# b0nes164/GPUSorting

Hardware: AMD Instinct MI355X
Metric: GKeys/s uint32 OneSweep at 1/2/4/8 MI355X; % HBM-read roofline (higher is better)
Workload: dtype u32; 1 GPU; 2^28 uniform-random uint32 keys-only OneSweep, 1 MI355X (BASELINE configs[1]); keys_per_gpu=268435456, entropy_preset=1, generator=InitRandom seed 10+i (+1000*rank), tile_keys=16384, verified_sorted=True

## Files before the change

### gpusorting_amd/csrc/hybrid_kernels.hpp

```cpp
#pragma once
#include "onesweep_kernels.hpp"
#include "mid_kernels.hpp"

namespace gs {

constexpr uint32_t HY_BINS = 65536;
constexpr uint32_t HY_JOINT_WORDS = HY_BINS / 2;
constexpr uint32_t HY_SLICE_WORDS = HY_JOINT_WORDS + RADIX;
constexpr uint32_t HY_VALID = 0;
constexpr uint32_t HY_MAXBUCKET = 1;
constexpr uint32_t HYT_JOINT = 0;
constexpr uint32_t HYT_BASE = HY_BINS;
constexpr uint32_t HYT_T = HYT_BASE + HY_BINS + 64;
constexpr uint32_t HYT_WORDS = HYT_T + NCH * RADIX;
static_assert(HYT_BASE % 4 == 0 && HYT_T % 4 == 0, "16-byte accesses");

constexpr int HY_HIST_THREADS = 1024;
constexpr uint32_t HY_FOLD_CHUNKS = 256;

template <int KT>
__global__ __launch_bounds__(HY_HIST_THREADS, HY_HIST_THREADS / 256) void hy_histogram_kernel(
    const uint32_t* __restrict__ keys, uint32_t* slab, size_t slab_used_words, uint32_t n, uint32_t seg_len0, uint32_t per_wg,
    uint32_t wg_per_seg, uint32_t* slices, uint32_t cap ) {
    static_assert(KeyWords<KT>::value == 1, "32-bit keys");
    constexpr uint32_t T = HY_HIST_THREADS;
    __shared__ __attribute__((aligned(16))) uint32_t s_j[HY_JOINT_WORDS];
    __shared__ __attribute__((aligned(16))) uint32_t s_r[RADIX / 2 * 32];
    __shared__ uint32_t s_b0[RADIX];
    __shared__ uint32_t s_red[4];
    const uint32_t tid = threadIdx.x, lane = tid & 63u;
    uint32_t* hist = slab + SLAB_HIST;
    {
        uint4* a = reinterpret_cast<uint4*>(slab);
        const size_t na = SLAB_HIST / 4, b0 = SLAB_HSUB / 4, nb = slab_used_words / 4;
        const size_t stride = (size_t)gridDim.x * T;
        const uint4 z = {0u, 0u, 0u, 0u};
        for (size_t i = (size_t)blockIdx.x * T + tid; i < na; i += stride) a[i] = z;
        for (size_t i = b0 + (size_t)blockIdx.x * T + tid; i < nb; i += stride) a[i] = z;
    }
    for (uint32_t i = tid; i < HY_JOINT_WORDS / 4; i += T) reinterpret_cast<uint4*>(s_j)[i] = uint4{0u, 0u, 0u, 0u};
    for (uint32_t i = tid; i < RADIX / 2 * 32 / 4; i += T) reinterpret_cast<uint4*>(s_r)[i] = uint4{0u, 0u, 0u, 0u};
    if (tid < RADIX) s_b0[tid] = 0;
    if (tid < 4) s_red[tid] = 0;
    auto fold = [&]() {
        __syncthreads();
        for (uint32_t i = tid; i < RADIX / 2 * 8; i += T) {
            const uint4 v = reinterpret_cast<const uint4*>(s_r)[i];
            reinterpret_cast<uint4*>(s_r)[i] = uint4{0u, 0u, 0u, 0u};
            uint32_t lo = (v.x & 0xffffu) + (v.y & 0xffffu) + (v.z & 0xffffu) + (v.w & 0xffffu);
            uint32_t hi = (v.x >> 16) + (v.y >> 16) + (v.z >> 16) + (v.w >> 16);
#pragma unroll
            for (int m = 1; m < 8; m <<= 1) {
                lo += __shfl_xor(lo, m, 64);
                hi += __shfl_xor(hi, m, 64);
            }
            if ((i & 7u) == 0u) {
                s_b0[(i >> 3) * 2u] += lo;
                s_b0[(i >> 3) * 2u + 1u] += hi;
            }
        }
        __syncthreads();
    };
    __syncthreads();

    const uint32_t x = blockIdx.x / wg_per_seg, jr = blockIdx.x % wg_per_seg;
    const unsigned long long sb = (unsigned long long)x * seg_len0, se = sb + seg_len0;
    const uint32_t seg_begin = sb < n ? (uint32_t)sb : n, seg_end = se < n ? (uint32_t)se : n;
    const unsigned long long rb = (unsigned long long)seg_begin + (unsigned long long)jr * per_wg;
    const uint32_t begin = rb < seg_end ? (uint32_t)rb : seg_end;
    const uint32_t end = (unsigned long long)begin + per_wg < seg_end ? begin + per_wg : seg_end;

    uint32_t k_or = 0, k_nand = 0;
    bool skew = false;
    uint32_t sticky = 0xffffffffu;
    uint32_t since_fold = 0;
    bool joint_off = false;
    typedef uint32_t hv4 __attribute__((ext_vector_type(4)));
    auto ld16 = [](const uint32_t* q) -> uint4 {
        const hv4 v = __builtin_nontemporal_load(reinterpret_cast<const hv4*>(q));
        return uint4{v.x, v.y, v.z, v.w};
    };
    auto add_joint = [&](uint32_t p, uint32_t c) { atomicAdd(&s_j[p >> 1], c << ((p & 1u) << 4)); };
    auto process = [&](const uint4 t, const bool probe) {
        const uint32_t b[4] = {t.x, t.y, t.z, t.w};
        k_or |= t.x | t.y | t.z | t.w;
        k_nand |= ~(t.x & t.y & t.z & t.w);
        if (since_fold >= HY_FOLD_CHUNKS) {
            fold();
            since_fold = 0;
        }
        ++since_fold;
#pragma unroll
        for (int j = 0; j < 4; ++j) {
            const uint32_t d = b[j] & 255u;
            atomicAdd(&s_r[(d >> 1) * 32u + (lane & 31u)], 1u << ((d & 1u) * 16u));
        }
        if (joint_off) return;
        if (probe) {
            const uint32_t p0 = b[0] >> 16;
            const uint32_t f = (uint32_t)__builtin_amdgcn_readfirstlane((int)p0);
            const uint32_t pc = (uint32_t)__popcll(__builtin_amdgcn_ballot_w64(p0 == f));
            if (pc >= HIST_SKEW_LANES) {
                skew = true;
                if (pc >= 24 || sticky == 0xffffffffu) sticky = f;
            }
        }
        if (!skew) {
#pragma unroll
            for (int j = 0; j < 4; ++j) add_joint(b[j] >> 16, 1u);
            return;
        }
        const uint32_t f = (uint32_t)__builtin_amdgcn_readfirstlane((int)(b[0] >> 16));
        const uint32_t pc = (uint32_t)__popcll(__builtin_amdgcn_ballot_w64((b[0] >> 16) == f));
        if (pc >= 24 && f != sticky) sticky = f;
        if (__builtin_amdgcn_ballot_w64((b[0] >> 16) == sticky && (b[1] >> 16) == sticky && (b[2] >> 16) == sticky && (b[3] >> 16) == sticky) == ~0ull) {
            if (lane == 0) add_joint(sticky, 256u);
            return;
        }
        uint32_t hit = 0;
#pragma unroll
        for (int j = 0; j < 4; ++j) {
            const uint32_t p = b[j] >> 16;
            const unsigned long long m = __builtin_amdgcn_ballot_w64(p == sticky);
            hit += (uint32_t)__popcll(m);
            if (p != sticky) add_joint(p, 1u);
            else if (__builtin_amdgcn_mbcnt_hi((uint32_t)(m >> 32), __builtin_amdgcn_mbcnt_lo((uint32_t)m, 0u)) == 0u)
                add_joint(sticky, (uint32_t)__popcll(m));
        }
        if (hit < 32) {
            sticky = f;
            if (pc < 8) skew = false;
        }
    };
    constexpr uint32_t UNROLL = HY_HIST_UNROLL;
    for (uint32_t c0 = begin; c0 < end; c0 += UNROLL * HIST_CHUNK) {
        if ((unsigned long long)c0 + UNROLL * HIST_CHUNK <= end) {
            uint4 t[UNROLL];
#pragma unroll
            for (uint32_t u = 0; u < UNROLL; ++u) t[u] = ld16(keys + c0 + u * HIST_CHUNK + tid * 4u);
            if (!joint_off) {
                const uint32_t pf = to_bits<KT>((uint32_t)__builtin_amdgcn_readfirstlane((int)t[0].x)) >> 16;
                if (lane == 0 && (((s_j[pf >> 1] >> ((pf & 1u) << 4)) & 0xffffu) > cap ||
                                  (skew && ((s_j[sticky >> 1] >> ((sticky & 1u) << 4)) & 0xffffu) > cap))) s_red[3] = 1u;
                joint_off = __builtin_amdgcn_readfirstlane((int)s_red[3]) != 0;
            }
#pragma unroll
            for (uint32_t u = 0; u < UNROLL; ++u)
                process(uint4{to_bits<KT>(t[u].x), to_bits<KT>(t[u].y), to_bits<KT>(t[u].z), to_bits<KT>(t[u].w)}, u == 0);
            continue;
        }
        for (uint32_t c = c0; c < end; c += HIST_CHUNK) {
            if ((unsigned long long)c + HIST_CHUNK <= end) {
                const uint4 t = ld16(keys + c + tid * 4u);
                process(uint4{to_bits<KT>(t.x), to_bits<KT>(t.y), to_bits<KT>(t.z), to_bits<KT>(t.w)}, true);
            } else {
                for (uint32_t i = c + tid; i < end; i += T) {
                    const uint32_t kb = to_bits<KT>(keys[i]);
                    k_or |= kb;
                    k_nand |= ~kb;
                    add_joint(kb >> 16, 1u);
                    atomicAdd(&s_b0[kb & 255u], 1u);
                }
            }
        }
    }
    fold();
    uint32_t* mine = slices + (size_t)blockIdx.x * HY_SLICE_WORDS;
    uint32_t sum = 0;
    for (uint32_t i = tid; i < HY_JOINT_WORDS / 4; i += T) {
        const uint4 v = reinterpret_cast<const uint4*>(s_j)[i];
        reinterpret_cast<uint4*>(mine)[i] = v;
        sum += (v.x & 0xffffu) + (v.x >> 16) + (v.y & 0xffffu) + (v.y >> 16) + (v.z & 0xffffu) + (v.z >> 16) + (v.w & 0xffffu) + (v.w >> 16);
    }
    if (tid < RADIX) mine[HY_JOINT_WORDS + tid] = s_b0[tid];
    sum = wave_reduce_sum(sum);
#pragma unroll
    for (int dd = 32; dd > 0; dd >>= 1) {
        k_or |= __shfl_xor(k_or, dd, 64);
        k_nand |= __shfl_xor(k_nand, dd, 64);
    }
    if (lane == 0) {
        atomicAdd(&s_red[0], sum);
        atomicOr(&s_red[1], k_or);
        atomicOr(&s_red[2], k_nand);
    }
    __syncthreads();
    if (tid == 0) {
        if (s_red[0] != end - begin || s_red[3] != 0u) atomicOr(&hist[HIST_TABLE_WORDS + HX_HY_BAD], 1u);
        atomicOr(&hist[HIST_TABLE_WORDS + HX_OR], s_red[1]);
        atomicOr(&hist[HIST_TABLE_WORDS + HX_NAND], s_red[2]);
    }
}

__global__ __launch_bounds__(256) void hy_reduce_kernel(const uint32_t* __restrict__ slices, uint32_t G, uint32_t wg_per_seg,
                                                         uint32_t* __restrict__ tab, uint32_t* __restrict__ hist) {
    __shared__ uint32_t s_acc[RADIX], s_T[NCH];
    const uint32_t tid = threadIdx.x;
    if (blockIdx.x >= RADIX) {
        const uint32_t x = blockIdx.x - RADIX;
        uint32_t acc = 0;
        for (uint32_t w = x * wg_per_seg; w < (x + 1u) * wg_per_seg && w < G; ++w) acc += slices[(size_t)w * HY_SLICE_WORDS + HY_JOINT_WORDS + tid];
        hist[hist_index(0, tid, x)] = acc;
        return;
    }
    const uint32_t b3 = blockIdx.x, w4 = tid & 31u, grp = tid >> 5;
    s_acc[tid] = 0;
    if (tid < NCH) s_T[tid] = 0;
    __syncthreads();
    uint32_t a[8] = {0u, 0u, 0u, 0u, 0u, 0u, 0u, 0u}, cur_x = 0xffffffffu, acc_x = 0;
    constexpr uint32_t U = 16;
    for (uint32_t s0 = grp; s0 < G; s0 += 8u * U) {
        uint4 v[U];
#pragma unroll
        for (uint32_t k = 0; k < U; ++k) {
            const uint32_t sl = s0 + 8u * k;
            v[k] = *reinterpret_cast<const uint4*>(slices + (size_t)(sl < G ? sl : G - 1u) * HY_SLICE_WORDS + b3 * 128u + w4 * 4u);
        }
#pragma unroll
        for (uint32_t k = 0; k < U; ++k) {
            const uint32_t sl = s0 + 8u * k;
            if (sl < G) {
                const uint32_t xs = sl / wg_per_seg;
                if (xs != cur_x) {
                    if (acc_x) atomicAdd(&s_T[cur_x], acc_x);
                    cur_x = xs;
                    acc_x = 0;
                }
                const uint32_t h[8] = {v[k].x & 0xffffu, v[k].x >> 16, v[k].y & 0xffffu, v[k].y >> 16, v[k].z & 0xffffu, v[k].z >> 16, v[k].w & 0xffffu, v[k].w >> 16};
#pragma unroll
                for (int j = 0; j < 8; ++j) { a[j] += h[j]; acc_x += h[j]; }
            }
        }
    }
    if (acc_x) atomicAdd(&s_T[cur_x], acc_x);
#pragma unroll
    for (int j = 0; j < 8; ++j) atomicAdd(&s_acc[w4 * 8u + j], a[j]);
    __syncthreads();
    tab[HYT_JOINT + b3 * RADIX + tid] = s_acc[tid];
    if (tid < NCH) tab[HYT_T + tid * RADIX + b3] = s_T[tid];
}

__global__ __launch_bounds__(1024) void hy_scan_kernel(uint32_t* slab, uint32_t* tab, uint32_t n, uint32_t seg_len0, uint32_t desc_stride,
                                                        uint32_t cap, uint32_t tile, uint32_t pregrouped ) {
    __shared__ uint32_t s_wt[RADIX];
    __shared__ uint32_t s_wmax[16], s_c4[4], s_rw[4];
    __shared__ uint32_t s_bstart[RADIX + 1], s_rowbase[RADIX];
    const uint32_t tid = threadIdx.x, lane = tid & 63u, wave = tid >> 6;
    uint32_t* hist = slab + SLAB_HIST;
    uint4 v[16];
#pragma unroll
    for (int i = 0; i < 16; ++i) v[i] = reinterpret_cast<const uint4*>(tab + HYT_JOINT)[i * 1024 + tid];
    uint32_t incl[16], mx = 0;
#pragma unroll
    for (int i = 0; i < 16; ++i) {
        const uint32_t s4 = v[i].x + v[i].y + v[i].z + v[i].w;
        const uint32_t m01 = v[i].x > v[i].y ? v[i].x : v[i].y, m23 = v[i].z > v[i].w ? v[i].z : v[i].w, m = m01 > m23 ? m01 : m23;
        mx = m > mx ? m : mx;
        incl[i] = wave_inclusive_scan_dpp(s4);
        if (lane == 63) s_wt[i * 16 + wave] = incl[i];
    }
#pragma unroll
    for (int dd = 32; dd > 0; dd >>= 1) {
        const uint32_t o = (uint32_t)__shfl_xor((int)mx, dd, 64);
        mx = o > mx ? o : mx;
    }
    if (lane == 0) s_wmax[wave] = mx;
    __syncthreads();
    uint32_t cv = 0, cincl = 0;
    if (tid < RADIX) {
        cv = s_wt[tid];
        cincl = wave_inclusive_scan_dpp(cv);
        if (lane == 63) s_c4[wave] = cincl;
    }
    __syncthreads();
    uint32_t total = 0, maxb = 0;
    for (uint32_t w = 0; w < 4; ++w) total += s_c4[w];
    for (uint32_t w = 0; w < 16; ++w) maxb = s_wmax[w] > maxb ? s_wmax[w] : maxb;
    if (tid < RADIX) {
        uint32_t b = cincl - cv;
        for (uint32_t w = 0; w < wave; ++w) b += s_c4[w];
        s_wt[tid] = b;
    }
    const bool valid = hist[HIST_TABLE_WORDS + HX_HY_BAD] == 0u && maxb <= cap && total == n;
    if (tid == 0) slab[SLAB_HY + HY_MAXBUCKET] = maxb;
    if (!valid) {
        if (tid == 0) hist[HIST_TABLE_WORDS + HX_SKEW] = 1u;
        return;
    }
    __syncthreads();
    uint32_t tseg[NCH];
#pragma unroll
    for (uint32_t x = 0; x < NCH; ++x) tseg[x] = tid < RADIX ? tab[HYT_T + x * RADIX + tid] : 0u;
#pragma unroll
    for (int i = 0; i < 16; ++i) {
        const uint4 c = v[i];
        const uint32_t e = s_wt[i * 16 + wave] + incl[i] - (c.x + c.y + c.z + c.w);
        v[i] = uint4{e, e + c.x, e + c.x + c.y, e + c.x + c.y + c.z};
        reinterpret_cast<uint4*>(tab + HYT_BASE)[i * 1024 + tid] = v[i];
        if (lane == 0) s_bstart[i * 16 + wave] = e;
    }
    if (tid == 0) {
        s_bstart[RADIX] = n;
        tab[HYT_BASE + HY_BINS] = n;
    }
    __syncthreads();
    uint32_t* info0 = slab + SLAB_INFO;
    uint32_t* info1 = info0 + INFO_STRIDE;
    uint32_t* desc0 = slab + SLAB_DESC;
    uint32_t* desc1 = desc0 + desc_stride;
    uint32_t rows = 0, rincl = 0;
    if (tid < RADIX) {
        rows = chain_tiles(s_bstart[tid], s_bstart[tid + 1], tile) + 1u;
        rincl = wave_inclusive_scan_dpp(rows);
        if (lane == 63) s_rw[wave] = rincl;
    }
    __syncthreads();
    if (tid < RADIX) {
        uint32_t rb = rincl - rows;
        for (uint32_t w = 0; w < wave; ++w) rb += s_rw[w];
        s_rowbase[tid] = rb;
        info1[I_START + tid] = s_bstart[tid];
        info1[I_END + tid] = s_bstart[tid + 1];
        info1[I_ROW + tid] = rb;
    }
    __syncthreads();
#pragma unroll
    for (int i = 0; i < 16; ++i) {
        uint4* row = reinterpret_cast<uint4*>(desc1 + (size_t)s_rowbase[i * 16 + wave] * RADIX);
        row[lane] = uint4{(v[i].x << 2) | FLAG_INCLUSIVE, (v[i].y << 2) | FLAG_INCLUSIVE, (v[i].z << 2) | FLAG_INCLUSIVE, (v[i].w << 2) | FLAG_INCLUSIVE};
    }
    if (tid < RADIX) {
        uint32_t run = s_bstart[tid], rowa = 0;
#pragma unroll
        for (uint32_t x = 0; x < NCH; ++x) {
            const unsigned long long a = (unsigned long long)x * seg_len0, b = a + seg_len0;
            const uint32_t s0 = a < n ? (uint32_t)a : n, s1 = b < n ? (uint32_t)b : n;
            desc0[(size_t)rowa * RADIX + tid] = (run << 2) | FLAG_INCLUSIVE;
            run += tseg[x];
            if (tid == 0) {
                info0[I_START + x] = s0;
                info0[I_END + x] = s1;
                info0[I_ROW + x] = rowa;
            }
            rowa += chain_tiles(s0, s1, tile) + 1u;
        }
    }
    if (tid == 0) {
        info0[PASS_FLAGS] = pregrouped ? PF_SKIP : 0u;
        info0[I_NCH] = NCH;
        info0[I_NEXT_SHIFT] = 0xffffffffu;
        info0[I_SHIFT] = 24u;
        info0[I_MODE] = 0xffffffffu;
        info1[PASS_FLAGS] = PF_SRC_ALT | PF_LAST;
        info1[I_NCH] = CHMAX;
        info1[I_NEXT_SHIFT] = 0xffffffffu;
        info1[I_SHIFT] = 16u;
        info1[I_MODE] = 0xffffffffu;
        info0[2 * INFO_STRIDE + PASS_FLAGS] = PF_SKIP;
        info0[3 * INFO_STRIDE + PASS_FLAGS] = PF_SKIP;
        hist[HIST_TABLE_WORDS + HX_HY] = 1u;
        slab[SLAB_HY + HY_VALID] = 1u;
    }
}
static_assert(CHMAX == RADIX, "pass B: one chain per top-byte value");

template <int KT, int THREADS_, int KPT_>
__global__ __launch_bounds__(THREADS_) void hy_local_sort_kernel(uint32_t* keys, const uint32_t* __restrict__ tab, uint32_t* __restrict__ slab,
                                                                 uint32_t n, uint32_t descending) {
    constexpr int KPT = KPT_, WAVES = THREADS_ / 64;
    constexpr uint32_t THREADS = THREADS_, TILE = THREADS_ * KPT_;
    static_assert(THREADS >= RADIX && KPT % 2 == 0 && WAVES % 2 == 0 && TILE < 65536, "one digit per thread in the scans; ranks and counters are packed two per word");
    __shared__ __attribute__((aligned(16))) uint32_t s_stage[TILE];
    __shared__ uint32_t s_cnt[WAVES / 2 * RADIX];
    __shared__ uint32_t s_wtot[4];
    const uint32_t tid = threadIdx.x, lane = tid & 63u, wave = tid >> 6;
    const uint32_t valid = slab[SLAB_HY + HY_VALID], b_lo = tab[HYT_BASE + blockIdx.x], b_hi = tab[HYT_BASE + blockIdx.x + 1u];
    if (__builtin_amdgcn_readfirstlane((int)valid) == 0) return;
    const uint32_t start = b_lo, count = b_hi - b_lo;
    if (count == 0u || count > TILE || start > n || count > n - start) return;
    const uint32_t at = descending ? n - start - count : start;
    const uint32_t kpt = (uint32_t)__builtin_amdgcn_readfirstlane((int)((count + THREADS - 1u) / THREADS));
    const uint32_t my_base = wave * (64u * kpt) + lane;
    uint32_t key[KPT];
#pragma unroll
    for (int i = 0; i < KPT; ++i) {
        if ((uint32_t)i >= kpt) continue;
        const uint32_t slot = my_base + i * 64u;
        key[i] = keys[at + (slot < count ? slot : count - 1u)];
    }
    if (tid < RADIX) s_cnt[tid] = 0;
#pragma unroll
    for (int i = 0; i < KPT; ++i)
        if ((uint32_t)i < kpt) key[i] = to_bits<KT>(key[i]);
    __syncthreads();
    uint32_t off[KPT / 2];
#pragma unroll
    for (int i = 0; i < KPT / 2; ++i) off[i] = 0;
#pragma unroll
    for (int i = 0; i < KPT; ++i) {
        if ((uint32_t)i >= kpt) continue;
        if (my_base + i * 64u < count)
            off[i >> 1] |= __hip_atomic_fetch_add(&s_cnt[key[i] & 255u], 1u, __ATOMIC_RELAXED, __HIP_MEMORY_SCOPE_WORKGROUP) << (16 * (i & 1));
    }
    __syncthreads();
    uint32_t c = 0, scan_incl = 0;
    if (tid < RADIX) {
        c = s_cnt[tid];
        scan_incl = wave_inclusive_scan_dpp(c);
        if (lane == 63) s_wtot[wave] = scan_incl;
    }
    __syncthreads();
    if (tid < RADIX) {
        uint32_t wbase = 0;
        for (uint32_t w = 0; w < wave; ++w) wbase += s_wtot[w];
        s_cnt[tid] = wbase + scan_incl - c;
    }
    __syncthreads();
#pragma unroll
    for (int i = 0; i < KPT; ++i) {
        if ((uint32_t)i >= kpt) continue;
        if (my_base + i * 64u < count) s_stage[((off[i >> 1] >> (16 * (i & 1))) & 0xffffu) + s_cnt[key[i] & 255u]] = key[i];
    }
    __syncthreads();
#pragma unroll
    for (int i = 0; i < KPT; ++i) {
        if ((uint32_t)i >= kpt) continue;
        key[i] = s_stage[my_base + i * 64u];
    }
    for (uint32_t i = tid; i < WAVES / 2 * RADIX; i += THREADS) s_cnt[i] = 0;
    __syncthreads();
    const uint32_t wsh = (uint32_t)__builtin_amdgcn_readfirstlane((int)((wave & 1u) * 16u));
    uint32_t* wh = s_cnt + (wave >> 1) * RADIX;
#pragma unroll
    for (int i = 0; i < KPT / 2; ++i) off[i] = 0;
#pragma unroll
    for (int i = 0; i < KPT; ++i) {
        if ((uint32_t)i >= kpt) continue;
        if (my_base + i * 64u < count) {
            const uint32_t r = __hip_atomic_fetch_add(&wh[(key[i] >> 8) & 255u], 1u << wsh, __ATOMIC_RELAXED, __HIP_MEMORY_SCOPE_WORKGROUP);
            off[i >> 1] |= ((r >> wsh) & 0xffffu) << (16 * (i & 1));
        }
    }
    __syncthreads();
    uint32_t run = 0;
    if (tid < RADIX) {
#pragma unroll
        for (int p = 0; p < WAVES / 2; ++p) {
            const uint32_t c2 = s_cnt[p * RADIX + tid];
            s_cnt[p * RADIX + tid] = run | ((run + (c2 & 0xffffu)) << 16);
            run += (c2 & 0xffffu) + (c2 >> 16);
        }
        scan_incl = wave_inclusive_scan_dpp(run);
        if (lane == 63) s_wtot[wave] = scan_incl;
    }
    __syncthreads();
    if (tid < RADIX) {
        uint32_t wbase = 0;
        for (uint32_t w = 0; w < wave; ++w) wbase += s_wtot[w];
        const uint32_t dpre = wbase + scan_incl - run;
#pragma unroll
        for (int p = 0; p < WAVES / 2; ++p) s_cnt[p * RADIX + tid] += dpre * 0x10001u;
    }
    __syncthreads();
#pragma unroll
    for (int i = 0; i < KPT; ++i) {
        if ((uint32_t)i >= kpt) continue;
        if (my_base + i * 64u < count)
            s_stage[((off[i >> 1] >> (16 * (i & 1))) & 0xffffu) + ((wh[(key[i] >> 8) & 255u] >> wsh) & 0xffffu)] = key[i];
    }
    __syncthreads();
#pragma unroll
    for (int i = 0; i < KPT; ++i) {
        const uint32_t slot = my_base + i * 64u;
        if ((uint32_t)i < kpt && slot < count) keys[at + (descending ? count - 1u - slot : slot)] = from_bits<KT>(s_stage[slot]);
    }
}

template <int KT, int VB, int THREADS_, int KPT_>
__global__ __launch_bounds__(THREADS_) void hy_local_sort_pairs_kernel(uint32_t* keys, void* vals_, const uint32_t* __restrict__ tab,
                                                                       const uint32_t* __restrict__ slab, uint32_t n, uint32_t descending) {
    using V = typename ValT<VB>::type;
    constexpr int KPT = KPT_, WAVES = THREADS_ / 64;
    constexpr uint32_t THREADS = THREADS_, TILE = THREADS_ * KPT_;
    static_assert(THREADS >= RADIX && KPT % 2 == 0 && WAVES % 2 == 0 && TILE < 65536, "slots of origin and counters are 16-bit fields");
    __shared__ __attribute__((aligned(16))) unsigned char s_raw[TILE * (VB > 4 ? VB : 4)];
    __shared__ uint32_t s_cnt[WAVES / 2 * RADIX];
    __shared__ uint32_t s_wtot[4];
    uint32_t* s_stage = reinterpret_cast<uint32_t*>(s_raw);
    V* s_vstage = reinterpret_cast<V*>(s_raw);
    V* vals = reinterpret_cast<V*>(vals_);
    const uint32_t tid = threadIdx.x, lane = tid & 63u, wave = tid >> 6;
    const uint32_t valid = slab[SLAB_HY + HY_VALID], b_lo = tab[HYT_BASE + blockIdx.x], b_hi = tab[HYT_BASE + blockIdx.x + 1u];
    if (__builtin_amdgcn_readfirstlane((int)valid) == 0) return;
    const uint32_t start = b_lo, count = b_hi - b_lo;
    if (count == 0u || count > TILE || start > n || count > n - start) return;
    const uint32_t at = descending ? n - start - count : start;
    const uint32_t kpt = (uint32_t)__builtin_amdgcn_readfirstlane((int)((count + THREADS - 1u) / THREADS));
    const uint32_t my_base = wave * (64u * kpt) + lane;
    uint32_t key[KPT];
    V val[KPT];
#pragma unroll
    for (int i = 0; i < KPT; ++i) {
        if ((uint32_t)i >= kpt) continue;
        const uint32_t slot = my_base + i * 64u, cs = slot < count ? slot : count - 1u;
        const uint32_t pos = at + (descending ? count - 1u - cs : cs);
        key[i] = keys[pos];
        val[i] = vals[pos];
    }
    const uint32_t wsh = (uint32_t)__builtin_amdgcn_readfirstlane((int)((wave & 1u) * 16u));
    uint32_t* wh = s_cnt + (wave >> 1) * RADIX;
#pragma unroll
    for (int i = 0; i < KPT; ++i)
        if ((uint32_t)i < kpt) key[i] = (to_bits<KT>(key[i]) & 0xffffu) | ((my_base + i * 64u) << 16);
    uint32_t off[KPT / 2];
#pragma unroll 1
    for (uint32_t shift = 0; shift < 16; shift += 8) {
        for (uint32_t i = tid; i < WAVES / 2 * RADIX; i += THREADS) s_cnt[i] = 0;
        __syncthreads();
#pragma unroll
        for (int i = 0; i < KPT / 2; ++i) off[i] = 0;
#pragma unroll
        for (int i = 0; i < KPT; ++i) {
            if ((uint32_t)i >= kpt) continue;
            if (my_base + i * 64u < count) {
                const uint32_t r = __hip_atomic_fetch_add(&wh[(key[i] >> shift) & 255u], 1u << wsh, __ATOMIC_RELAXED, __HIP_MEMORY_SCOPE_WORKGROUP);
                off[i >> 1] |= ((r >> wsh) & 0xffffu) << (16 * (i & 1));
            }
        }
        __syncthreads();
        uint32_t run = 0, scan_incl = 0;
        if (tid < RADIX) {
#pragma unroll
            for (int p = 0; p < WAVES / 2; ++p) {
                const uint32_t c2 = s_cnt[p * RADIX + tid];
                s_cnt[p * RADIX + tid] = run | ((run + (c2 & 0xffffu)) << 16);
                run += (c2 & 0xffffu) + (c2 >> 16);
            }
            scan_incl = wave_inclusive_scan_dpp(run);
            if (lane == 63) s_wtot[wave] = scan_incl;
        }
        __syncthreads();
        if (tid < RADIX) {
            uint32_t wbase = 0;
            for (uint32_t w = 0; w < wave; ++w) wbase += s_wtot[w];
            const uint32_t dpre = wbase + scan_incl - run;
#pragma unroll
            for (int p = 0; p < WAVES / 2; ++p) s_cnt[p * RADIX + tid] += dpre * 0x10001u;
        }
        __syncthreads();
#pragma unroll
        for (int i = 0; i < KPT; ++i) {
            if ((uint32_t)i >= kpt) continue;
            if (my_base + i * 64u < count)
                s_stage[((off[i >> 1] >> (16 * (i & 1))) & 0xffffu) + ((wh[(key[i] >> shift) & 255u] >> wsh) & 0xffffu)] = key[i];
        }
        __syncthreads();
#pragma unroll
        for (int i = 0; i < KPT; ++i) {
            if ((uint32_t)i >= kpt) continue;
            key[i] = s_stage[my_base + i * 64u];
        }
    }
    __syncthreads();
#pragma unroll
    for (int i = 0; i < KPT; ++i) {
        if ((uint32_t)i >= kpt) continue;
        if (my_base + i * 64u < count) s_vstage[my_base + i * 64u] = val[i];
    }
    __syncthreads();
    const uint32_t top = blockIdx.x << 16;
#pragma unroll
    for (int i = 0; i < KPT; ++i) {
        const uint32_t slot = my_base + i * 64u;
        if ((uint32_t)i < kpt && slot < count) {
            const uint32_t pos = at + (descending ? count - 1u - slot : slot);
            keys[pos] = from_bits<KT>(top | (key[i] & 0xffffu));
            vals[pos] = s_vstage[key[i] >> 16];
        }
    }
}

__global__ __launch_bounds__(256) void hy_void_copy_kernel(const uint32_t* __restrict__ slab, const uint4* __restrict__ src, uint4* __restrict__ dst,
                                                            size_t words16, const uint32_t* __restrict__ src_tail, uint32_t* __restrict__ dst_tail,
                                                            uint32_t tail_words) {
    if (__builtin_amdgcn_readfirstlane((int)slab[SLAB_HY + HY_VALID]) != 0) return;
    const size_t stride = (size_t)gridDim.x * 256u;
    for (size_t i = (size_t)blockIdx.x * 256u + threadIdx.x; i < words16; i += stride) dst[i] = src[i];
    if (blockIdx.x == 0 && threadIdx.x < tail_words) dst_tail[threadIdx.x] = src_tail[threadIdx.x];
}

}
```

Before: 167.7 GKeys/s.

## Stage only low 16 bits of keys in LDS during hybrid local sort

```diff
diff --git a/gpusorting_amd/csrc/hybrid_kernels.hpp b/gpusorting_amd/csrc/hybrid_kernels.hpp
--- a/gpusorting_amd/csrc/hybrid_kernels.hpp
+++ b/gpusorting_amd/csrc/hybrid_kernels.hpp
@@ -367,38 +367,40 @@
 template <int KT, int THREADS_, int KPT_>
 __global__ __launch_bounds__(THREADS_) void hy_local_sort_kernel(uint32_t* keys, const uint32_t* __restrict__ tab, uint32_t* __restrict__ slab,
                                                                  uint32_t n, uint32_t descending) {
-    constexpr int KPT = KPT_, WAVES = THREADS_ / 64;
+    constexpr int KPT = KPT_, KP2 = KPT_ / 2, WAVES = THREADS_ / 64;
     constexpr uint32_t THREADS = THREADS_, TILE = THREADS_ * KPT_;
-    static_assert(THREADS >= RADIX && KPT % 2 == 0 && WAVES % 2 == 0 && TILE < 65536, "one digit per thread in the scans; ranks and counters are packed two per word");
-    __shared__ __attribute__((aligned(16))) uint32_t s_stage[TILE];
+    static_assert(THREADS >= RADIX && KPT % 2 == 0 && WAVES % 2 == 0 && TILE < 65536 && TILE % 128 == 0,
+                  "one digit per thread in the scans; ranks and counters are packed two per word; the stage is whole blocks of 128 halfwords");
+    __shared__ __attribute__((aligned(16))) uint32_t s_stage[TILE / 2 + 4];
     __shared__ uint32_t s_cnt[WAVES / 2 * RADIX];
     __shared__ uint32_t s_wtot[4];
+    uint16_t* s_half = reinterpret_cast<uint16_t*>(s_stage);
     const uint32_t tid = threadIdx.x, lane = tid & 63u, wave = tid >> 6;
     const uint32_t valid = slab[SLAB_HY + HY_VALID], b_lo = tab[HYT_BASE + blockIdx.x], b_hi = tab[HYT_BASE + blockIdx.x + 1u];
     if (__builtin_amdgcn_readfirstlane((int)valid) == 0) return;
     const uint32_t start = b_lo, count = b_hi - b_lo;
     if (count == 0u || count > TILE || start > n || count > n - start) return;
     const uint32_t at = descending ? n - start - count : start;
-    const uint32_t kpt = (uint32_t)__builtin_amdgcn_readfirstlane((int)((count + THREADS - 1u) / THREADS));
-    const uint32_t my_base = wave * (64u * kpt) + lane;
+    const uint32_t kp2 = (uint32_t)__builtin_amdgcn_readfirstlane((int)((count + 2u * THREADS - 1u) / (2u * THREADS)));
+    const uint32_t my_base = wave * (128u * kp2) + lane;
     uint32_t key[KPT];
 #pragma unroll
     for (int i = 0; i < KPT; ++i) {
-        if ((uint32_t)i >= kpt) continue;
+        if ((uint32_t)(i >> 1) >= kp2) continue;
         const uint32_t slot = my_base + i * 64u;
         key[i] = keys[at + (slot < count ? slot : count - 1u)];
     }
     if (tid < RADIX) s_cnt[tid] = 0;
 #pragma unroll
     for (int i = 0; i < KPT; ++i)
-        if ((uint32_t)i < kpt) key[i] = to_bits<KT>(key[i]);
+        if ((uint32_t)(i >> 1) < kp2) key[i] = to_bits<KT>(key[i]);
     __syncthreads();
     uint32_t off[KPT / 2];
 #pragma unroll
     for (int i = 0; i < KPT / 2; ++i) off[i] = 0;
 #pragma unroll
     for (int i = 0; i < KPT; ++i) {
-        if ((uint32_t)i >= kpt) continue;
+        if ((uint32_t)(i >> 1) >= kp2) continue;
         if (my_base + i * 64u < count)
             off[i >> 1] |= __hip_atomic_fetch_add(&s_cnt[key[i] & 255u], 1u, __ATOMIC_RELAXED, __HIP_MEMORY_SCOPE_WORKGROUP) << (16 * (i & 1));
     }
@@ -418,14 +420,18 @@
     __syncthreads();
 #pragma unroll
     for (int i = 0; i < KPT; ++i) {
-        if ((uint32_t)i >= kpt) continue;
-        if (my_base + i * 64u < count) s_stage[((off[i >> 1] >> (16 * (i & 1))) & 0xffffu) + s_cnt[key[i] & 255u]] = key[i];
-    }
-    __syncthreads();
-#pragma unroll
-    for (int i = 0; i < KPT; ++i) {
-        if ((uint32_t)i >= kpt) continue;
-        key[i] = s_stage[my_base + i * 64u];
+        if ((uint32_t)(i >> 1) >= kp2) continue;
+        if (my_base + i * 64u < count) {
+            const uint32_t r = ((off[i >> 1] >> (16 * (i & 1))) & 0xffffu) + s_cnt[key[i] & 255u];
+            s_half[(r & ~127u) | ((r & 63u) << 1) | ((r >> 6) & 1u)] = (uint16_t)key[i];
+        }
+    }
+    __syncthreads();
+    uint32_t kw[KP2];
+#pragma unroll
+    for (int j = 0; j < KP2; ++j) {
+        if ((uint32_t)j >= kp2) continue;
+        kw[j] = s_stage[wave * (64u * kp2) + j * 64u + lane];
     }
     for (uint32_t i = tid; i < WAVES / 2 * RADIX; i += THREADS) s_cnt[i] = 0;
     __syncthreads();
@@ -435,9 +441,10 @@
     for (int i = 0; i < KPT / 2; ++i) off[i] = 0;
 #pragma unroll
     for (int i = 0; i < KPT; ++i) {
-        if ((uint32_t)i >= kpt) continue;
+        if ((uint32_t)(i >> 1) >= kp2) continue;
         if (my_base + i * 64u < count) {
-            const uint32_t r = __hip_atomic_fetch_add(&wh[(key[i] >> 8) & 255u], 1u << wsh, __ATOMIC_RELAXED, __HIP_MEMORY_SCOPE_WORKGROUP);
+            const uint32_t d = (i & 1) ? kw[i >> 1] >> 24 : (kw[i >> 1] >> 8) & 255u;
+            const uint32_t r = __hip_atomic_fetch_add(&wh[d], 1u << wsh, __ATOMIC_RELAXED, __HIP_MEMORY_SCOPE_WORKGROUP);
             off[i >> 1] |= ((r >> wsh) & 0xffffu) << (16 * (i & 1));
         }
     }
@@ -462,18 +469,31 @@
         for (int p = 0; p < WAVES / 2; ++p) s_cnt[p * RADIX + tid] += dpre * 0x10001u;
     }
     __syncthreads();
-#pragma unroll
-    for (int i = 0; i < KPT; ++i) {
-        if ((uint32_t)i >= kpt) continue;
-        if (my_base + i * 64u < count)
-            s_stage[((off[i >> 1] >> (16 * (i & 1))) & 0xffffu) + ((wh[(key[i] >> 8) & 255u] >> wsh) & 0xffffu)] = key[i];
-    }
-    __syncthreads();
-#pragma unroll
-    for (int i = 0; i < KPT; ++i) {
-        const uint32_t slot = my_base + i * 64u;
-        if ((uint32_t)i < kpt && slot < count) keys[at + (descending ? count - 1u - slot : slot)] = from_bits<KT>(s_stage[slot]);
-    }
+    const uint32_t par = at & 1u, flip = descending ? 0xffffffffu : 0u, pos0 = par + (descending ? count - 1u : 0u);
+#pragma unroll
+    for (int i = 0; i < KPT; ++i) {
+        if ((uint32_t)(i >> 1) >= kp2) continue;
+        if (my_base + i * 64u < count) {
+            const uint32_t d = (i & 1) ? kw[i >> 1] >> 24 : (kw[i >> 1] >> 8) & 255u;
+            const uint32_t r = ((off[i >> 1] >> (16 * (i & 1))) & 0xffffu) + ((wh[d] >> wsh) & 0xffffu);
+            s_half[pos0 + ((r ^ flip) - flip)] = (uint16_t)((i & 1) ? kw[i >> 1] >> 16 : kw[i >> 1]);
+        }
+    }
+    __syncthreads();
+    const uint32_t top = blockIdx.x << 16, end = par + count;
+    uint32_t* out = keys + (at - par);
+    auto store_word = [&](const uint32_t m) {
+        const uint32_t w = s_stage[m], h0 = 2u * m;
+        const uint32_t k0 = from_bits<KT>(top | (w & 0xffffu)), k1 = from_bits<KT>(top | (w >> 16));
+        const bool v0 = h0 >= par && h0 < end, v1 = h0 + 1u < end;
+        if (v0 && v1) *reinterpret_cast<uint2*>(out + h0) = uint2{k0, k1};
+        else if (v0) out[h0] = k0;
+        else if (v1) out[h0 + 1u] = k1;
+    };
+#pragma unroll
+    for (int j = 0; j < KP2; ++j)
+        if ((uint32_t)j < kp2) store_word(tid + j * THREADS);
+    if (tid == 0u && end > 2u * kp2 * THREADS) store_word(kp2 * THREADS);
 }
 
 template <int KT, int VB, int THREADS_, int KPT_>
```

Measured after the change: 166.3 GKeys/s. No clear change (-0.9%).
